# risc0/zeth

Measured on AMD Instinct MI355X. Metric: segments/sec, higher is better.
Workload: dtype u32

## Files before the change

### zeth_amd/csrc/common.h

```cpp
#pragma once
#include <hip/hip_runtime.h>

#include <atomic>
#include <cstdarg>
#include <cstdio>
#include <cstdlib>
#include <cstring>
#include <map>
#include <string>
#include <vector>

#include "../../include/zkhal.h"
#include "fp.h"
#include "noise.h"

namespace zkh {

inline const char* make_err(const char* fmt, ...) {
    char buf[512];
    va_list ap;
    va_start(ap, fmt);
    vsnprintf(buf, sizeof buf, fmt, ap);
    va_end(ap);
    return strdup(buf);
}
#define ZKH_HIP(expr)                                                                               \
    do {                                                                                            \
        hipError_t _e = (expr);                                                                     \
        if (_e != hipSuccess) return zkh::make_err("%s failed: %s (%s:%d)", #expr, hipGetErrorString(_e), __FILE__, __LINE__); \
    } while (0)
#define ZKH_TRY(expr)                    \
    do {                                 \
        const char* _err = (expr);       \
        if (_err) return _err;           \
    } while (0)
#define ZKH_REQUIRE(cond, ...)                         \
    do {                                               \
        if (!(cond)) return zkh::make_err(__VA_ARGS__); \
    } while (0)

constexpr int ZKH_P2_PTAB = 414;
constexpr int TW_BITS = 12;
constexpr int TW_SIZE = 1 << TW_BITS;
constexpr int TW_HI_BITS = 14;
constexpr int TW_HI_SIZE = 1 << TW_HI_BITS;
constexpr int MAX_LOG_N = TW_BITS + TW_HI_BITS;
constexpr int LDS_TW_LOG = 12;

struct DeviceTables {
    uint32_t* rc;
    uint32_t* diag;
    uint32_t* tw_fwd_lo; uint32_t* tw_fwd_hi;
    uint32_t* tw_rev_lo; uint32_t* tw_rev_hi;
    uint32_t* tile_fwd;  uint32_t* tile_rev;
    uint32_t* layer_fwd; uint32_t* layer_rev;
    uint32_t* layer_fwd_plain;
    uint32_t* shift_lo;  uint32_t* shift_hi;
};

struct ProfAgg { uint64_t calls = 0; double ms = 0; double bytes = 0; };
struct ProfPending { std::string name; hipEvent_t a, b; double bytes; };

}

struct zkh_alloc_t {
    void* ptr;
    size_t bytes;
    std::atomic<int> refs;
    bool owned;
    zkh_ctx* ctx;
    zkh_alloc_t(void* p, size_t b, int r, bool o, zkh_ctx* c) : ptr(p), bytes(b), refs(r), owned(o), ctx(c) {}
};

struct zkh_buf {
    zkh_alloc_t* a;
    size_t off, len;
    std::atomic<int> refs;
    zkh_buf(zkh_alloc_t* al, size_t o, size_t l, int r) : a(al), off(o), len(l), refs(r) {}
    uint32_t* ptr() const { return (uint32_t*)a->ptr + off; }
};

struct zkh_ctx {
    int device;
    hipStream_t stream;
    zkh::DeviceTables tab;
    uint32_t rou_fwd[28], rou_rev[28];
    uint32_t h_rc[24 * 29], h_diag[zkh::ZKH_P2_PTAB];
    std::multimap<size_t, void*> pool;
    size_t pool_bytes = 0, live_bytes = 0, peak_bytes = 0;
    bool prof = false;
    std::vector<zkh::ProfPending> pending;
    std::map<std::string, zkh::ProfAgg> agg;
    std::vector<hipEvent_t> event_pool;
    uint32_t* pinned = nullptr;
    size_t pinned_words = 0;
    size_t stage_next = 0, stage_used = 0;
    uint32_t* d_fail = nullptr;
    uint32_t* h_fail = nullptr;
    bool fail_armed = false;
    std::map<void*, size_t> host_blocks;
};

namespace zkh {

const char* pool_alloc(zkh_ctx* c, size_t bytes, void** out);
void pool_free(zkh_ctx* c, void* p, size_t bytes);
const char* new_buf(zkh_ctx* c, size_t n_words, bool zero, zkh_buf** out);
void prof_begin(zkh_ctx* c, const char* name, double bytes);
void prof_end(zkh_ctx* c);
const char* ensure_pinned(zkh_ctx* c, size_t words);
const char* resolve_noise_key(const uint32_t* key_or_null, NoiseKey* out);

inline void bind_thread(const zkh_ctx* c) { (void)hipSetDevice(c->device); }
const char* ntt_device_init(zkh_ctx* c);

struct Tmp {
    zkh_buf* b = nullptr;
    Tmp() {}
    Tmp(const Tmp&) = delete;
    Tmp& operator=(const Tmp&) = delete;
    ~Tmp() { if (b) zkh_release(b); }
    zkh_buf** out() { if (b) { zkh_release(b); b = nullptr; } return &b; }
    operator zkh_buf*() const { return b; }
    zkh_buf* operator->() const { return b; }
    explicit operator bool() const { return b != nullptr; }
};

struct ProfScope {
    zkh_ctx* c;
    ProfScope(zkh_ctx* ctx, const char* name, double bytes) : c(ctx) { bind_thread(c); if (c->prof) prof_begin(c, name, bytes); }
    ~ProfScope() { if (c->prof) prof_end(c); }
};

inline const char* last_launch_error(const char* what) {
    hipError_t e = hipGetLastError();
    if (e != hipSuccess) return make_err("launch %s: %s", what, hipGetErrorString(e));
    return nullptr;
}

// ... 8 lines not shown
```

### zeth_amd/csrc/hal.hip

```cpp
#include <algorithm>

#include "common.h"

#include <sys/random.h>
#include "poseidon2.h"
#include "../../include/zkh_poseidon2_consts.h"

using namespace zkh;

extern "C" void zkh_free_error(const char* e) { free((void*)e); }
#if ZKH_P2_CONSTS_ARE_PLACEHOLDER
extern "C" const char* zkh_version(void) { return "zkhal-mi355x 0.2.0 (gfx950; poseidon2_consts=placeholder)"; }
#elif ZKH_P2_CONSTS_ARE_DERIVED
extern "C" const char* zkh_version(void) { return "zkhal-mi355x 0.2.0 (gfx950; poseidon2_consts=derived)"; }
#else
extern "C" const char* zkh_version(void) { return "zkhal-mi355x 0.2.0 (gfx950; poseidon2_consts=upstream)"; }
#endif

namespace zkh {

const char* pool_alloc(zkh_ctx* c, size_t bytes, void** out) {
    bytes = (bytes + 255) & ~(size_t)255;
    if (bytes == 0) bytes = 256;
    auto it = c->pool.find(bytes);
    if (it != c->pool.end()) {
        *out = it->second;
        c->pool.erase(it);
        c->pool_bytes -= bytes;
    } else {
        hipError_t e = hipMalloc(out, bytes);
        if (e != hipSuccess) {
            (void)hipStreamSynchronize(c->stream);
            for (auto& kv : c->pool) (void)hipFree(kv.second);
            c->pool.clear(); c->pool_bytes = 0;
            e = hipMalloc(out, bytes);
            if (e != hipSuccess) return make_err("hipMalloc(%zu) failed: %s", bytes, hipGetErrorString(e));
        }
    }
    c->live_bytes += bytes;
    if (c->live_bytes > c->peak_bytes) c->peak_bytes = c->live_bytes;
    return nullptr;
}
void pool_free(zkh_ctx* c, void* p, size_t bytes) {
    bytes = (bytes + 255) & ~(size_t)255;
    if (bytes == 0) bytes = 256;
    c->live_bytes -= bytes;
    c->pool.emplace(bytes, p);
    c->pool_bytes += bytes;
}
const char* new_buf(zkh_ctx* c, size_t n_words, bool zero, zkh_buf** out) {
    bind_thread(c);
    void* p = nullptr;
    ZKH_TRY(pool_alloc(c, n_words * 4, &p));
    if (zero && n_words) {
        hipError_t e = hipMemsetAsync(p, 0, n_words * 4, c->stream);
        if (e != hipSuccess) return make_err("hipMemsetAsync: %s", hipGetErrorString(e));
    }
    zkh_alloc_t* a = new zkh_alloc_t(p, n_words * 4, 1, true, c);
    *out = new zkh_buf(a, 0, n_words, 1);
    return nullptr;
}
const char* ensure_pinned(zkh_ctx* c, size_t words) {
    if (c->pinned_words >= words) return nullptr;
    if (c->pinned) (void)hipHostFree(c->pinned);
    size_t w = words < 65536 ? 65536 : words;
    ZKH_HIP(hipHostMalloc((void**)&c->pinned, w * 4, hipHostMallocDefault));
    c->pinned_words = w;
    return nullptr;
}
static hipEvent_t get_event(zkh_ctx* c) {
    if (!c->event_pool.empty()) { hipEvent_t e = c->event_pool.back(); c->event_pool.pop_back(); return e; }
    hipEvent_t e;
    (void)hipEventCreate(&e);
    return e;
}
void prof_begin(zkh_ctx* c, const char* name, double bytes) {
    ProfPending p{name, get_event(c), get_event(c), bytes};
    (void)hipEventRecord(p.a, c->stream);
    c->pending.push_back(p);
}
void prof_end(zkh_ctx* c) { (void)hipEventRecord(c->pending.back().b, c->stream); }
static void prof_flush(zkh_ctx* c) {
    if (c->pending.empty()) return;
    (void)hipStreamSynchronize(c->stream);
    for (auto& p : c->pending) {
        float ms = 0;
        (void)hipEventElapsedTime(&ms, p.a, p.b);
        auto& g = c->agg[p.name];
// ... 16 lines not shown
    for (int tries = 0; tries < 4 && !ok; tries++) {
        ok = getrandom(out->k, sizeof out->k, 0) == (ssize_t)sizeof out->k;
        bool nonzero = false;
        for (int i = 0; i < 8; i++) nonzero = nonzero || out->k[i] != 0;
        ok = ok && nonzero;
    }
    ZKH_REQUIRE(ok, "OS randomness (getrandom) is unavailable: refusing to seal with a predictable blinding key");
    return nullptr;
}
extern "C" uint32_t zkh_noise_cell_host(const uint32_t noise_key[8], uint32_t group, uint32_t column, uint32_t row) {
    NoiseKey k;
    memcpy(k.k, noise_key, sizeof k.k);
    return noise_cell(k, group, column, row);
}
extern "C" void zkh_chacha_block_host(const uint32_t key[8], const uint32_t counter_nonce[4], int double_rounds, uint32_t out[16]) {
    chacha_block(key, counter_nonce[0], counter_nonce[1], counter_nonce[2], counter_nonce[3], double_rounds, out, 16);
}
static std::vector<uint32_t> powers(Fp base, size_t n) {
    std::vector<uint32_t> v(n);
    Fp cur = Fp::one();
    for (size_t i = 0; i < n; i++) { v[i] = cur.v; cur = cur * base; }
    return v;
}

}

extern "C" const char* zkh_poseidon2_set_constants(zkh_ctx* c, const uint32_t* rc, const uint32_t* diag) {
    bind_thread(c);
    std::vector<uint32_t> r(24 * 29), d(ZKH_P2_PTAB);
    for (int i = 0; i < 24 * 29; i++) r[i] = fp_encode(rc[i]).v - P;
    poseidon2_partial_table(d.data(), rc, diag);
    memcpy(c->h_rc, r.data(), sizeof c->h_rc);
    memcpy(c->h_diag, d.data(), sizeof c->h_diag);
    ZKH_HIP(hipStreamSynchronize(c->stream));
    ZKH_HIP(hipMemcpy(c->tab.rc, r.data(), r.size() * 4, hipMemcpyHostToDevice));
    ZKH_HIP(hipMemcpy(c->tab.diag, d.data(), d.size() * 4, hipMemcpyHostToDevice));
    return nullptr;
}

static const char* ctx_init_tables(zkh_ctx* c);
extern "C" const char* zkh_ctx_create(int device, const char* suite, zkh_ctx** out) {
    ZKH_REQUIRE(suite && strcmp(suite, "poseidon2") == 0, "unsupported hash suite '%s' (only poseidon2)", suite ? suite : "(null)");
    int ndev = 0;
    hipError_t e = hipGetDeviceCount(&ndev);
    ZKH_REQUIRE(e == hipSuccess && ndev > 0, "no HIP device available (%s): libzkhal_mi355x has no CPU fallback",
                e == hipSuccess ? "device count 0" : hipGetErrorString(e));
    ZKH_REQUIRE(device >= 0 && device < ndev, "device ordinal %d out of range (%d devices)", device, ndev);
    ZKH_HIP(hipSetDevice(device));
    zkh_ctx* c = new zkh_ctx();
    c->device = device;
    if (hipError_t se = hipStreamCreateWithFlags(&c->stream, hipStreamNonBlocking); se != hipSuccess) {
        delete c;
        return make_err("hipStreamCreateWithFlags: %s", hipGetErrorString(se));
    }
    if (const char* err = ctx_init_tables(c)) {
        zkh_ctx_destroy(c);
        return err;
    }
    *out = c;
    return nullptr;
}
static const char* ctx_init_tables(zkh_ctx* c) {
    Fp g = fp_encode(137);
    for (int k = 0; k <= 27; k++) {
        Fp w = fp_pow(g, 1ull << (27 - k));
        c->rou_fwd[k] = w.v;
        c->rou_rev[k] = fp_inv(w).v;
    }
    Fp wf = Fp::raw(c->rou_fwd[MAX_LOG_N]), wr = Fp::raw(c->rou_rev[MAX_LOG_N]);
    ZKH_TRY(upload(&c->tab.tw_fwd_lo, powers(wf, TW_SIZE)));
    ZKH_TRY(upload(&c->tab.tw_fwd_hi, powers(fp_pow(wf, TW_SIZE), TW_HI_SIZE)));
    ZKH_TRY(upload(&c->tab.tw_rev_lo, powers(wr, TW_SIZE)));
    ZKH_TRY(upload(&c->tab.tw_rev_hi, powers(fp_pow(wr, TW_SIZE), TW_HI_SIZE)));
    ZKH_TRY(upload(&c->tab.tile_fwd, powers(Fp::raw(c->rou_fwd[LDS_TW_LOG]), 1 << (LDS_TW_LOG - 1))));
    ZKH_TRY(upload(&c->tab.tile_rev, powers(Fp::raw(c->rou_rev[LDS_TW_LOG]), 1 << (LDS_TW_LOG - 1))));
    {
        std::vector<uint32_t> lf(1 << LDS_TW_LOG, R1), lr(1 << LDS_TW_LOG, R1);
        for (int j = 1; j <= LDS_TW_LOG; j++) {
            auto pf = powers(Fp::raw(c->rou_fwd[j]), (size_t)1 << (j - 1)), pr = powers(Fp::raw(c->rou_rev[j]), (size_t)1 << (j - 1));
            for (size_t e = 0; e < pf.size(); e++) { lf[((size_t)1 << (j - 1)) + e] = pf[e]; lr[((size_t)1 << (j - 1)) + e] = pr[e]; }
        }
        ZKH_TRY(upload(&c->tab.layer_fwd, lf));
        ZKH_TRY(upload(&c->tab.layer_rev, lr));
        for (auto& w : lf) w = mont_reduce((uint64_t)w);
        ZKH_TRY(upload(&c->tab.layer_fwd_plain, lf));
    }
    Fp three = fp_encode(3);
    ZKH_TRY(upload(&c->tab.shift_lo, powers(three, TW_SIZE)));
    ZKH_TRY(upload(&c->tab.shift_hi, powers(fp_pow(three, TW_SIZE), TW_HI_SIZE)));
    ZKH_TRY(upload(&c->tab.rc, std::vector<uint32_t>(24 * 29)));
    ZKH_TRY(upload(&c->tab.diag, std::vector<uint32_t>(ZKH_P2_PTAB)));
    ZKH_TRY(zkh_poseidon2_set_constants(c, ZKH_P2_ROUND_CONSTANTS, ZKH_P2_M_INT_DIAG));
    ZKH_TRY(ntt_device_init(c));
    ZKH_HIP(hipMalloc((void**)&c->d_fail, 8));
    ZKH_HIP(hipMemsetAsync(c->d_fail, 0, 8, c->stream));
    ZKH_HIP(hipHostMalloc((void**)&c->h_fail, 8, hipHostMallocDefault));
    c->h_fail[0] = c->h_fail[1] = 0;
    return nullptr;
}
extern "C" const char* zkh_ctx_trim(zkh_ctx* c) {
    bind_thread(c);
    ZKH_HIP(hipStreamSynchronize(c->stream));
    for (auto& kv : c->pool) (void)hipFree(kv.second);
    c->pool.clear(); c->pool_bytes = 0;
    return nullptr;
}
extern "C" void zkh_ctx_memory(const zkh_ctx* c, size_t* live, size_t* cached, size_t* peak) {
    if (live) *live = c->live_bytes;
    if (cached) *cached = c->pool_bytes;
    if (peak) *peak = c->peak_bytes;
}
extern "C" void zkh_ctx_destroy(zkh_ctx* c) {
    if (!c) return;
    (void)hipSetDevice(c->device);
    (void)hipStreamSynchronize(c->stream);
    for (auto& kv : c->pool) (void)hipFree(kv.second);
    uint32_t* t[] = {c->tab.rc, c->tab.diag, c->tab.tw_fwd_lo, c->tab.tw_fwd_hi, c->tab.tw_rev_lo, c->tab.tw_rev_hi,
                     c->tab.tile_fwd, c->tab.tile_rev, c->tab.shift_lo, c->tab.shift_hi, c->tab.layer_fwd, c->tab.layer_rev, c->tab.layer_fwd_plain};
    for (auto p : t) (void)hipFree(p);
    for (auto& p : c->pending) { (void)hipEventDestroy(p.a); (void)hipEventDestroy(p.b); }
    for (auto ev : c->event_pool) (void)hipEventDestroy(ev);
    if (c->pinned) (void)hipHostFree(c->pinned);
    if (c->d_fail) (void)hipFree(c->d_fail);
    if (c->h_fail) (void)hipHostFree(c->h_fail);
    for (auto& kv : c->host_blocks) (void)hipHostFree(kv.first);
    (void)hipStreamDestroy(c->stream);
    delete c;
}
static const char* check_device_fail(zkh_ctx* c) {
    if (!c->fail_armed) return nullptr;
    c->fail_armed = false;
    const uint32_t code = c->h_fail[0], detail = c->h_fail[1];
    if (!code) return nullptr;
    (void)hipMemsetAsync(c->d_fail, 0, 8, c->stream);
    switch (code) {
    case 1: return make_err("combos_prepare_regs: register %u has size 0 or more than `cycles` words (found on the device; the call's combos are unchanged)", detail);
    case 2: return make_err("combos_prepare_regs: register %u names a combo beyond combo_count (found on the device; the call's combos are unchanged)", detail);
    case 3: return make_err("combos_prepare_regs: the register sizes add up to %u U coefficients (+ %d of the check polynomial), more than coeff_u holds (found on the device; the call's combos are unchanged)", detail, ZKH_CHECK_SIZE);
    default: return make_err("a kernel reported failure code %u (%u)", code, detail);
    }
}
static const char* sync_checked(zkh_ctx* c) {
    if (c->fail_armed) ZKH_HIP(hipMemcpyAsync(c->h_fail, c->d_fail, 8, hipMemcpyDeviceToHost, c->stream));
    ZKH_HIP(hipStreamSynchronize(c->stream));
    c->stage_used = 0;
    return check_device_fail(c);
}
extern "C" const char* zkh_sync(zkh_ctx* c) {
    bind_thread(c);
    return sync_checked(c);
}
extern "C" void* zkh_ctx_stream(zkh_ctx* c) { return (void*)c->stream; }

extern "C" const char* zkh_alloc(zkh_ctx* c, const char*, size_t n, int zero, zkh_buf** out) {
    return new_buf(c, n, zero != 0, out);
}
namespace zkh {
constexpr size_t STAGE_SLOT_WORDS = 16384, STAGE_SLOTS = 64;
const char* h2d(zkh_ctx* c, uint32_t* dst, const uint32_t* host, size_t n) {
    if (!n) return nullptr;
    bind_thread(c);
    if (n <= STAGE_SLOT_WORDS) {
        ZKH_TRY(ensure_pinned(c, STAGE_SLOT_WORDS * STAGE_SLOTS));
        if (c->stage_used == STAGE_SLOTS) ZKH_TRY(sync_checked(c));
        uint32_t* slot = c->pinned + (size_t)c->stage_next * STAGE_SLOT_WORDS;
        memcpy(slot, host, n * 4);
        ZKH_HIP(hipMemcpyAsync(dst, slot, n * 4, hipMemcpyHostToDevice, c->stream));
        c->stage_next = (c->stage_next + 1) % STAGE_SLOTS;
        c->stage_used++;
        return nullptr;
    }
    ZKH_HIP(hipMemcpyAsync(dst, host, n * 4, hipMemcpyHostToDevice, c->stream));
    return sync_checked(c);
}
}
extern "C" const char* zkh_copy_from(zkh_ctx* c, const char*, const uint32_t* host, size_t n, zkh_buf** out) {
    ZKH_TRY(new_buf(c, n, false, out));
    return h2d(c, (*out)->ptr(), host, n);
}
extern "C" const char* zkh_wrap(zkh_ctx* c, void* dptr, size_t n, zkh_buf** out) {
    zkh_alloc_t* a = new zkh_alloc_t(dptr, n * 4, 1, false, c);
    *out = new zkh_buf(a, 0, n, 1);
    return nullptr;
}
extern "C" const char* zkh_slice(zkh_buf* b, size_t off, size_t n, zkh_buf** out) {
    ZKH_REQUIRE(n <= b->len && off <= b->len - n, "slice [%zu, +%zu) out of range (size %zu)", off, n, b->len);
    b->a->refs.fetch_add(1, std::memory_order_relaxed);
    *out = new zkh_buf(b->a, b->off + off, n, 1);
    return nullptr;
}
extern "C" void zkh_retain(zkh_buf* b) { b->refs.fetch_add(1, std::memory_order_relaxed); }
extern "C" void zkh_release(zkh_buf* b) {
    if (!b || b->refs.fetch_sub(1, std::memory_order_acq_rel) > 1) return;
    zkh_alloc_t* a = b->a;
    if (a->refs.fetch_sub(1, std::memory_order_acq_rel) == 1) {
        if (a->owned) pool_free(a->ctx, a->ptr, a->bytes);
        delete a;
    }
    delete b;
}
extern "C" size_t zkh_size(const zkh_buf* b) { return b->len; }
// ... 313 lines not shown
```

### zeth_amd/csrc/ntt.hip

```cpp
#include "common.h"

using namespace zkh;

namespace {

constexpr int NTT_THREADS = 256;

struct PassParams {
    const uint32_t* in;
    uint32_t* out;
    size_t in_col_stride;
    size_t out_col_stride;
    uint32_t log_n;
    uint32_t L, R;
    uint32_t log_t;
    uint32_t expand_bits;
    uint32_t first_layer;
    uint32_t twiddle;
    uint32_t scale;
    uint32_t zk_shift;
    const uint32_t* tile_tw;
    const uint32_t* layer_tw;
    const uint32_t* tw_lo;
    const uint32_t* tw_hi;
    const uint32_t* sh_lo;
    const uint32_t* sh_hi;
    uint32_t tiles_per_col;
    uint32_t lazy;
    uint32_t lazy_comp;
    uint32_t shift16[16];
};

template <bool INVERSE>
__global__ __launch_bounds__(NTT_THREADS) void k_ntt_pass(PassParams p) {
    extern __shared__ __attribute__((aligned(16))) uint32_t tile[];
    const uint32_t T = 1u << p.log_t, rows = 1u << p.R, elems = rows << p.log_t;
    const uint32_t tid = threadIdx.x;
    const uint32_t tile_id = xcd_remap(blockIdx.x, p.tiles_per_col);
    const uint32_t col = blockIdx.y;
    const uint32_t ltiles = 1u << (p.L - p.log_t);
    const uint32_t a = tile_id >> (p.L - p.log_t), lt = tile_id & (ltiles - 1);
    const size_t base = ((size_t)a << (p.L + p.R)) + ((size_t)lt << p.log_t);
    const uint32_t l0 = lt << p.log_t;
    const uint32_t* in = p.in + (size_t)col * p.in_col_stride;
    uint32_t* out = p.out + (size_t)col * p.out_col_stride;
    const uint32_t tw_shift = MAX_LOG_N - (p.L + p.R);

    for (uint32_t e = tid; e < elems; e += NTT_THREADS) {
        const uint32_t m = e >> p.log_t, t = e & (T - 1);
        const size_t gi = base + ((size_t)m << p.L) + t;
        uint32_t v = in[gi >> p.expand_bits];
        if (!INVERSE && p.twiddle) {
            const uint32_t r = __brev(m) >> (32 - p.R);
            const uint32_t ex = ((l0 + t) * r) << tw_shift;
            const uint32_t w = mul_mod(p.tw_lo[ex & (TW_SIZE - 1)], p.tw_hi[ex >> TW_BITS]);
            v = mul_mod(v, w);
        }
        tile[e] = v;
    }
    __syncthreads();

    const uint32_t half_elems = elems >> 1;
    if (INVERSE) {
        for (uint32_t j = p.R; j >= 1; j--) {
            const uint32_t hb = j - 1;
            for (uint32_t q = tid; q < half_elems; q += NTT_THREADS) {
                const uint32_t t = q & (T - 1), mm = q >> p.log_t;
                const uint32_t low = mm & ((1u << hb) - 1), m = ((mm >> hb) << j) | low;
                const uint32_t i0 = (m << p.log_t) | t, i1 = i0 + (1u << (hb + p.log_t));
                const uint32_t x = tile[i0], y = tile[i1];
                const uint32_t w = p.tile_tw[low << (LDS_TW_LOG - j)];
                tile[i0] = add_mod(x, y);
                tile[i1] = mul_mod(x - y + P, w);
            }
            __syncthreads();
        }
    } else {
        for (uint32_t j = p.first_layer; j <= p.R; j++) {
            const uint32_t hb = j - 1;
            for (uint32_t q = tid; q < half_elems; q += NTT_THREADS) {
                const uint32_t t = q & (T - 1), mm = q >> p.log_t;
                const uint32_t low = mm & ((1u << hb) - 1), m = ((mm >> hb) << j) | low;
                const uint32_t i0 = (m << p.log_t) | t, i1 = i0 + (1u << (hb + p.log_t));
// ... 73 lines not shown
                const int low = i0 & ((1 << hb) - 1), i1 = i0 + (1 << hb);
                const uint32_t w = low ? p.tile_tw[(uint32_t)low << (LDS_TW_LOG - j)] : 0u;
#pragma unroll
                for (int c = 0; c < 4; c++) {
                    const uint32_t x = v[i0][c], y = low ? mul_mod(v[i1][c], w) : v[i1][c];
                    v[i0][c] = add_mod(x, y);
                    v[i1][c] = sub_mod(x, y);
                }
            }
        }
    } else {
#pragma unroll
        for (int j = R; j >= 1; j--) {
            const int hb = j - 1;
#pragma unroll
            for (int i0 = 0; i0 < N; i0++) {
                if (i0 & (1 << hb)) continue;
                const int low = i0 & ((1 << hb) - 1), i1 = i0 + (1 << hb);
                const uint32_t w = low ? p.tile_tw[(uint32_t)low << (LDS_TW_LOG - j)] : 0u;
#pragma unroll
                for (int c = 0; c < 4; c++) {
                    const uint32_t x = v[i0][c], y = v[i1][c];
                    v[i0][c] = add_mod(x, y);
                    v[i1][c] = low ? mul_mod(x - y + P, w) : sub_mod(x, y);
                }
            }
        }
        four_step();
    }
#pragma unroll
    for (int m = 0; m < N; m++) *(uint4*)(out + ((size_t)m << p.L)) = make_uint4(v[m][0], v[m][1], v[m][2], v[m][3]);
}

__global__ void k_zk_shift(uint32_t* io, size_t total, uint32_t log_n, const uint32_t* sh_lo, const uint32_t* sh_hi) {
    size_t i = (size_t)blockIdx.x * blockDim.x + threadIdx.x;
    if (i >= total) return;
    const uint32_t pos = (uint32_t)(i & (((size_t)1 << log_n) - 1));
    const uint32_t ex = log_n ? __brev(pos) >> (32 - log_n) : 0;
    io[i] = mul_mod(io[i], mul_mod(sh_lo[ex & (TW_SIZE - 1)], sh_hi[ex >> TW_BITS]));
}

constexpr int BR_H = 5;
__global__ __launch_bounds__(256) void k_bit_reverse_tiled(uint32_t* io, uint32_t log_n, size_t col_stride) {
    __shared__ uint32_t ta[1 << (2 * BR_H)], tb[1 << (2 * BR_H)];
    const uint32_t mid_bits = log_n - 2 * BR_H;
    const uint32_t mid = blockIdx.x;
    const uint32_t rmid = mid_bits ? __brev(mid) >> (32 - mid_bits) : 0;
    if (rmid < mid) return;
    uint32_t* col = io + (size_t)blockIdx.y * col_stride;
    const uint32_t H = 1u << BR_H;
    for (uint32_t e = threadIdx.x; e < H * H; e += blockDim.x) {
        const uint32_t hi = e >> BR_H, lo = e & (H - 1);
        ta[e] = col[((size_t)hi << (log_n - BR_H)) | ((size_t)mid << BR_H) | lo];
        if (rmid != mid) tb[e] = col[((size_t)hi << (log_n - BR_H)) | ((size_t)rmid << BR_H) | lo];
    }
    __syncthreads();
    for (uint32_t e = threadIdx.x; e < H * H; e += blockDim.x) {
        const uint32_t hi2 = e >> BR_H, lo2 = e & (H - 1);
        const uint32_t shi = __brev(lo2) >> (32 - BR_H), slo = __brev(hi2) >> (32 - BR_H);
        const uint32_t src = (shi << BR_H) | slo;
        col[((size_t)hi2 << (log_n - BR_H)) | ((size_t)rmid << BR_H) | lo2] = ta[src];
        if (rmid != mid) col[((size_t)hi2 << (log_n - BR_H)) | ((size_t)mid << BR_H) | lo2] = tb[src];
    }
}
__global__ void k_bit_reverse_small(uint32_t* io, uint32_t log_n, size_t count) {
    size_t g = (size_t)blockIdx.x * blockDim.x + threadIdx.x;
    size_t n = (size_t)1 << log_n;
    if (g >= n * count) return;
    uint32_t i = (uint32_t)(g & (n - 1));
    uint32_t r = log_n ? __brev(i) >> (32 - log_n) : 0;
    if (i < r) {
        uint32_t* col = io + (g - i);
        uint32_t x = col[i], y = col[r];
        col[i] = y; col[r] = x;
    }
}


template <int LOGR, bool INVERSE, bool BASE0, int J_LO, bool LAZY = false>
__device__ __forceinline__ void radix_layers(uint32_t (&v)[1 << LOGR], const uint32_t* __restrict__ ltab,
                                             const uint32_t base_low, const int first_b) {
    constexpr int N = 1 << LOGR;
    if (!INVERSE && LAZY) {
#pragma unroll
        for (int b = 0; b < LOGR; b++) {
            if (b < first_b) continue;
            const uint32_t* tw = ltab + (1u << (J_LO + b - 1));
#pragma unroll
            for (int kk = 0; kk < (1 << b); kk++) {
                const bool unit = BASE0 && kk == 0;
                const int32_t w = (int32_t)(unit ? 1u : tw[base_low + ((uint32_t)kk << (J_LO - 1))]), nw = -w;
#pragma unroll
                for (int hi = 0; hi < (N >> (b + 1)); hi++) {
                    const int k = (hi << (b + 1)) | kk;
                    const int64_t x = (int64_t)(int32_t)v[k];
                    const int32_t y = (int32_t)v[k + (1 << b)];
                    v[k] = (uint32_t)smont_reduce(BASE0 ? mad_i64_k(y, w, x) : mad_i64(y, w, x));
                    v[k + (1 << b)] = (uint32_t)smont_reduce(BASE0 ? mad_i64_k(y, nw, x) : mad_i64(y, nw, x));
                }
            }
        }
    } else if (INVERSE) {
#pragma unroll
        for (int b = LOGR - 1; b >= 0; b--) {
            const uint32_t* tw = ltab + (1u << (J_LO + b - 1));
#pragma unroll
            for (int kk = 0; kk < (1 << b); kk++) {
                const bool unit = BASE0 && kk == 0;
                const uint32_t w = unit ? 0u : tw[base_low + ((uint32_t)kk << (J_LO - 1))];
#pragma unroll
                for (int hi = 0; hi < (N >> (b + 1)); hi++) {
                    const int k = (hi << (b + 1)) | kk;
                    const uint32_t x = v[k], y = v[k + (1 << b)];
                    v[k] = add_mod(x, y);
                    v[k + (1 << b)] = unit ? sub_mod(x, y) : mul_mod(x - y + P, w);
                }
            }
        }
    } else {
#pragma unroll
        for (int b = 0; b < LOGR; b++) {
            if (b < first_b) continue;
            const uint32_t* tw = ltab + (1u << (J_LO + b - 1));
#pragma unroll
            for (int kk = 0; kk < (1 << b); kk++) {
                const bool unit = BASE0 && kk == 0;
                const uint32_t w = unit ? 0u : tw[base_low + ((uint32_t)kk << (J_LO - 1))];
#pragma unroll
                for (int hi = 0; hi < (N >> (b + 1)); hi++) {
                    const int k = (hi << (b + 1)) | kk;
                    const uint32_t x = v[k], y = unit ? v[k + (1 << b)] : mul_mod(v[k + (1 << b)], w);
                    v[k] = add_mod(x, y);
                    v[k + (1 << b)] = sub_mod(x, y);
                }
            }
        }
    }
}

template <bool INVERSE, bool LAZY = false>
__global__ __launch_bounds__(256) void k_ntt_low12(PassParams p) {
    __shared__ __attribute__((aligned(16))) uint32_t lds[4096];
    const uint32_t tid = threadIdx.x;
    const uint32_t tile = xcd_remap(blockIdx.x, p.tiles_per_col);
    const size_t base = (size_t)tile << 12;
    const uint32_t* in = p.in + (size_t)blockIdx.y * p.in_col_stride;
    uint32_t* out = p.out + (size_t)blockIdx.y * p.out_col_stride;
    const uint32_t* __restrict__ ltab = p.layer_tw;
    const uint32_t hi = tid >> 4, low = tid & 15;
    uint32_t v[16];
    if (INVERSE) {
#pragma unroll
        for (int k = 0; k < 16; k++) v[k] = in[base + k * 256 + tid];
        radix_layers<4, true, false, 9>(v, ltab, tid, 0);
#pragma unroll
        for (int k = 0; k < 16; k++) lds[k * 256 + tid] = v[k];
        __syncthreads();
#pragma unroll
        for (int k = 0; k < 16; k++) v[k] = lds[hi * 256 + k * 16 + low];
        radix_layers<4, true, false, 5>(v, ltab, low, 0);
#pragma unroll
        for (int k = 0; k < 16; k++) lds[hi * 256 + k * 16 + low] = v[k];
        __syncthreads();
#pragma unroll
        for (int q = 0; q < 4; q++) {
            const uint4 w = ((const uint4*)lds)[tid * 4 + q];
            v[4 * q] = w.x; v[4 * q + 1] = w.y; v[4 * q + 2] = w.z; v[4 * q + 3] = w.w;
        }
        radix_layers<4, true, true, 1>(v, ltab, 0, 0);
        const size_t pos0 = base + (size_t)tid * 16;
        if (p.zk_shift) {
            const uint32_t ex = __brev((uint32_t)pos0) >> (32 - p.log_n);
            const uint32_t b = mul_mod(p.sh_lo[ex & (TW_SIZE - 1)], p.sh_hi[ex >> TW_BITS]);
#pragma unroll
            for (int k = 0; k < 16; k++) v[k] = mul_mod(mul_mod(v[k], b), p.shift16[k]);
        } else if (p.scale) {
#pragma unroll
            for (int k = 0; k < 16; k++) v[k] = mul_mod(v[k], p.scale);
        }
#pragma unroll
        for (int q = 0; q < 4; q++) ((uint4*)(out + pos0))[q] = make_uint4(v[4 * q], v[4 * q + 1], v[4 * q + 2], v[4 * q + 3]);
    } else {
        const size_t pos0 = base + (size_t)tid * 16;
        if (p.expand_bits == 0) {
// ... 118 lines not shown
                radix_layers<2, false, true, 1, LAZY>(u, ltab, 0, 0);
#pragma unroll
                for (int k = 0; k < 4; k++) lds[(m0 + k) * TW + t] = u[k];
            }
            __syncthreads();
#pragma unroll
            for (int k = 0; k < 16; k++) v[k] = lds[(hi * 64 + k * 4 + low) * TW + t];
            radix_layers<4, false, false, 3, LAZY>(v, ltab, low, 0);
#pragma unroll
            for (int k = 0; k < 16; k++) lds[(hi * 64 + k * 4 + low) * TW + t] = v[k];
            __syncthreads();
#pragma unroll
            for (int k = 0; k < 16; k++) v[k] = lds[(k * 64 + g) * TW + t];
            radix_layers<4, false, false, 7, LAZY>(v, ltab, g, 0);
#pragma unroll
            for (int k = 0; k < 16; k++) TILE_OUT(k * 64 + g) = LAZY ? canon((int32_t)v[k]) : v[k];
        }
    } else {
        if (INVERSE) {
#pragma unroll
            for (int k = 0; k < 16; k++) v[k] = TILE_IN(k * 16 + g);
            radix_layers<4, true, false, 5>(v, ltab, g, 0);
#pragma unroll
            for (int k = 0; k < 16; k++) lds[(k * 16 + g) * TW + t] = v[k];
            __syncthreads();
#pragma unroll
            for (int k = 0; k < 16; k++) v[k] = lds[(g * 16 + k) * TW + t];
            radix_layers<4, true, true, 1>(v, ltab, 0, 0);
#pragma unroll
            for (int k = 0; k < 16; k++) {
                uint32_t x = mul_mod(v[k], tw[k]);
                if (p.scale) x = mul_mod(x, p.scale);
                TILE_OUT(g * 16 + k) = x;
            }
        } else {
#pragma unroll
            for (int k = 0; k < 16; k++) {
                const uint32_t x = TILE_IN(g * 16 + k);
                v[k] = LAZY ? (uint32_t)smont((int32_t)x, (int32_t)tw[k]) : mul_mod(x, tw[k]);
            }
            radix_layers<4, false, true, 1, LAZY>(v, ltab, 0, 0);
#pragma unroll
            for (int k = 0; k < 16; k++) lds[(g * 16 + k) * TW + t] = v[k];
            __syncthreads();
#pragma unroll
            for (int k = 0; k < 16; k++) v[k] = lds[(k * 16 + g) * TW + t];
            radix_layers<4, false, false, 5, LAZY>(v, ltab, g, 0);
#pragma unroll
            for (int k = 0; k < 16; k++) TILE_OUT(k * 16 + g) = LAZY ? canon((int32_t)v[k]) : v[k];
        }
    }
}
#undef TILE_IN
#undef TILE_OUT

struct Pass { uint32_t L, R; };
std::vector<Pass> plan_passes(uint32_t log_n) {
    std::vector<Pass> v;
    if (log_n <= 12) { v.push_back({0, log_n}); return v; }
    if (log_n < 18) {
        const uint32_t low = (log_n + 1) / 2;
        v.push_back({0, low});
        v.push_back({low, log_n - low});
        return v;
    }
    const uint32_t rem = log_n - 12;
    v.push_back({0, 12});
    if (rem == 8 || rem == 10 || rem <= 7) v.push_back({12, rem});
    else if (rem == 9) { v.push_back({12, 8}); v.push_back({20, 1}); }
    else if (rem == 11 || rem == 12) { v.push_back({12, 8}); v.push_back({20, rem - 8}); }
    else { v.push_back({12, 10}); v.push_back({22, rem - 10}); }
    return v;
}

const char* run_transform(zkh_ctx* c, bool inverse, const uint32_t* in, size_t in_col_stride, uint32_t* out,
                          size_t out_col_stride, uint32_t log_n, size_t count, uint32_t expand_bits, bool zk, const char* name) {
    ZKH_REQUIRE(log_n <= (uint32_t)MAX_LOG_N, "%s: transform size 2^%u exceeds the supported 2^%d", name, log_n, MAX_LOG_N);
    ZKH_REQUIRE(count <= 65535, "%s: too many columns (%zu)", name, count);
    std::vector<Pass> passes = plan_passes(log_n);
    const size_t n = (size_t)1 << log_n;
    Fp ninv = fp_inv(fp_encode((uint32_t)(n % P)));
    const size_t npass = passes.size();
    const bool lazy = !inverse && npass == 2 && passes[0].R == 12 && (passes[1].R == 8 || passes[1].R == 10) && expand_bits <= 4;
    const uint32_t lazy_comp = lazy ? fp_pow(Fp::raw(R2), passes[0].R - expand_bits + passes[1].R).v : 0;
    for (size_t pi = 0; pi < npass; pi++) {
        const Pass ps = inverse ? passes[npass - 1 - pi] : passes[pi];
        PassParams p{};
        const bool first = pi == 0, last = pi + 1 == npass;
        p.in = first ? in : out;
        p.in_col_stride = first ? in_col_stride : out_col_stride;
        p.out = out; p.out_col_stride = out_col_stride;
        p.log_n = log_n; p.L = ps.L; p.R = ps.R;
        const bool reg_high = ps.L >= 4 && (ps.R == 8 || ps.R == 10);
        p.log_t = ps.L == 0 ? 0 : (ps.L < 4 ? ps.L : 4);
        if (ps.L != 0 && !reg_high && ps.R < 12) p.log_t = std::max<uint32_t>(p.log_t, std::min<uint32_t>(ps.L, 12 - ps.R));
        while (p.R + p.log_t > 14 && p.log_t > 0) p.log_t--;
        p.expand_bits = (!inverse && first) ? expand_bits : 0;
        p.first_layer = (!inverse && first) ? expand_bits + 1 : 1;
        p.twiddle = ps.L != 0;
        p.scale = (inverse && last) ? ninv.v : 0;
        p.zk_shift = (inverse && last && zk) ? 1 : 0;
        p.lazy = lazy; p.lazy_comp = lazy_comp;
        p.tile_tw = inverse ? c->tab.tile_rev : c->tab.tile_fwd;
        p.layer_tw = inverse ? c->tab.layer_rev : (lazy ? c->tab.layer_fwd_plain : c->tab.layer_fwd);
        p.tw_lo = inverse ? c->tab.tw_rev_lo : c->tab.tw_fwd_lo;
        p.tw_hi = inverse ? c->tab.tw_rev_hi : c->tab.tw_fwd_hi;
        p.sh_lo = c->tab.shift_lo; p.sh_hi = c->tab.shift_hi;
        if (p.zk_shift && log_n >= 4) {
            const Fp three = fp_encode(3);
            for (uint32_t k = 0; k < 16; k++)
                p.shift16[k] = (ninv * fp_pow(three, (uint64_t)(bitrev32(k) >> 28) << (log_n - 4))).v;
        }
        p.tiles_per_col = (uint32_t)(n >> (p.R + p.log_t));
        const size_t lds = ((size_t)4 << (p.R + p.log_t));
        dim3 grid(p.tiles_per_col, (unsigned)count);
        const double alg_bytes = pi == 0 ? 4.0 * count * (double)(((size_t)1 << log_n) >> expand_bits) + 4.0 * count * (double)n : 0.0;
        const bool scale_here = p.scale != 0;
        const bool k_low = ps.L == 0 && ps.R == 12 && p.expand_bits <= 4;
        const bool k_h10 = !k_low && ps.L >= 4 && p.log_t == 4 && ps.R == 10 && !(scale_here && p.zk_shift);
        const bool k_h8 = !k_low && !k_h10 && ps.L >= 4 && p.log_t == 4 && ps.R == 8 && !(scale_here && p.zk_shift);
        const bool k_top = !k_low && !k_h10 && !k_h8 && ps.L >= 12 && ps.L + ps.R == log_n && ps.R >= 1 && ps.R <= 4 && p.twiddle &&
                           p.expand_bits == 0 && p.first_layer == 1 && !scale_here && !p.zk_shift;
        const std::string pname = std::string(name) + (k_low ? ":k_ntt_low12" : k_h10 ? ":k_ntt_high10" : k_h8 ? ":k_ntt_high8" : k_top ? ":k_ntt_top" : ":k_ntt_pass");
        ProfScope prof(c, pname.c_str(), alg_bytes);
        if (ps.L == 0 && ps.R == 12 && p.expand_bits <= 4) {
            if (inverse) k_ntt_low12<true><<<grid, 256, 0, c->stream>>>(p);
            else if (lazy) k_ntt_low12<false, true><<<grid, 256, 0, c->stream>>>(p);
            else k_ntt_low12<false><<<grid, 256, 0, c->stream>>>(p);
        } else if (ps.L >= 4 && p.log_t == 4 && ps.R == 10 && !(scale_here && p.zk_shift)) {
            if (inverse) k_ntt_high<10, true><<<grid, 1024, lds, c->stream>>>(p);
            else if (lazy) k_ntt_high<10, false, true><<<grid, 1024, lds, c->stream>>>(p);
            else k_ntt_high<10, false><<<grid, 1024, lds, c->stream>>>(p);
        } else if (ps.L >= 4 && p.log_t == 4 && ps.R == 8 && !(scale_here && p.zk_shift)) {
            if (inverse) k_ntt_high<8, true><<<grid, 256, lds, c->stream>>>(p);
            else if (lazy) k_ntt_high<8, false, true><<<grid, 256, lds, c->stream>>>(p);
            else k_ntt_high<8, false><<<grid, 256, lds, c->stream>>>(p);
        } else if (k_top) {
            const dim3 tg((unsigned)(((size_t)1 << ps.L) >> 10), (unsigned)count);
            switch (ps.R * 2 + (inverse ? 1 : 0)) {
            case 2: k_ntt_top<1, false><<<tg, 256, 0, c->stream>>>(p); break;
            case 3: k_ntt_top<1, true><<<tg, 256, 0, c->stream>>>(p); break;
            case 4: k_ntt_top<2, false><<<tg, 256, 0, c->stream>>>(p); break;
            case 5: k_ntt_top<2, true><<<tg, 256, 0, c->stream>>>(p); break;
            case 6: k_ntt_top<3, false><<<tg, 256, 0, c->stream>>>(p); break;
            case 7: k_ntt_top<3, true><<<tg, 256, 0, c->stream>>>(p); break;
            case 8: k_ntt_top<4, false><<<tg, 256, 0, c->stream>>>(p); break;
            default: k_ntt_top<4, true><<<tg, 256, 0, c->stream>>>(p); break;
            }
        } else if (inverse) k_ntt_pass<true><<<grid, NTT_THREADS, lds, c->stream>>>(p);
        else k_ntt_pass<false><<<grid, NTT_THREADS, lds, c->stream>>>(p);
        ZKH_TRY(last_launch_error(name));
    }
    return nullptr;
}

}

const char* zkh::ntt_device_init(zkh_ctx* c) {
    bind_thread(c);
    ZKH_HIP(hipFuncSetAttribute((const void*)k_ntt_high<10, true>, hipFuncAttributeMaxDynamicSharedMemorySize, 65536));
    ZKH_HIP(hipFuncSetAttribute((const void*)k_ntt_high<10, false>, hipFuncAttributeMaxDynamicSharedMemorySize, 65536));
    ZKH_HIP(hipFuncSetAttribute((const void*)k_ntt_high<10, false, true>, hipFuncAttributeMaxDynamicSharedMemorySize, 65536));
    return nullptr;
}

static const char* interpolate_impl(zkh_ctx* c, zkh_buf* io, size_t count, bool zk, const char* name) {
    ZKH_REQUIRE(count && io->len % count == 0, "%s: size %zu not a multiple of count %zu", name, io->len, count);
    const size_t n = io->len / count;
    const uint32_t log_n = log2_ceil(n);
    ZKH_REQUIRE(((size_t)1 << log_n) == n, "%s: column length %zu is not a power of two", name, n);
    return run_transform(c, true, io->ptr(), n, io->ptr(), n, log_n, count, 0, zk, name);
}
extern "C" const char* zkh_batch_interpolate_ntt(zkh_ctx* c, zkh_buf* io, size_t count) {
    return interpolate_impl(c, io, count, false, "batch_interpolate_ntt");
}
extern "C" const char* zkh_batch_interpolate_ntt_zk_shift(zkh_ctx* c, zkh_buf* io, size_t count) {
    return interpolate_impl(c, io, count, true, "batch_interpolate_ntt_zk_shift");
}
extern "C" const char* zkh_batch_interpolate_ntt_from(zkh_ctx* c, zkh_buf* out, const zkh_buf* in, size_t count, int zk_shift) {
    ZKH_REQUIRE(count && in->len % count == 0 && out->len == in->len, "batch_interpolate_ntt_from: shape mismatch");
    const size_t n = in->len / count;
    const uint32_t log_n = log2_ceil(n);
    ZKH_REQUIRE(((size_t)1 << log_n) == n, "batch_interpolate_ntt_from: column length %zu is not a power of two", n);
    return run_transform(c, true, in->ptr(), n, out->ptr(), n, log_n, count, 0, zk_shift != 0, "batch_interpolate_ntt_from");
}
extern "C" const char* zkh_batch_expand_into_evaluate_ntt(zkh_ctx* c, zkh_buf* out, const zkh_buf* in, size_t count,
                                                          size_t expand_bits) {
// ... 36 lines not shown
```

Measured before the change: 42.80.

## Fuse pairs of lazy NTT butterfly layers to halve Montgomery reductions

Reworks the lazy forward NTT radix layers to process two butterfly layers at once. The first layer's sums stay as unreduced 64-bit accumulators and get folded into the second layer's multiply-add, so only one signed Montgomery reduction happens per two layers. A new twiddle table holds centered plain and Montgomery-form twiddles for this, and the compensation power of R is recomputed from the new reduction count. This cuts the ALU work spent on reductions, at the cost of wider intermediate values and extra twiddle loads, with some overflow risk in the unreduced sums.

```diff
diff --git a/zeth_amd/csrc/common.h b/zeth_amd/csrc/common.h
--- a/zeth_amd/csrc/common.h
+++ b/zeth_amd/csrc/common.h
@@ -54,7 +54,7 @@
     uint32_t* tw_rev_lo; uint32_t* tw_rev_hi;
     uint32_t* tile_fwd;  uint32_t* tile_rev;
     uint32_t* layer_fwd; uint32_t* layer_rev;
-    uint32_t* layer_fwd_plain;
+    uint32_t* layer_fwd_lazy;
     uint32_t* shift_lo;  uint32_t* shift_hi;
 };
 
diff --git a/zeth_amd/csrc/hal.hip b/zeth_amd/csrc/hal.hip
--- a/zeth_amd/csrc/hal.hip
+++ b/zeth_amd/csrc/hal.hip
@@ -4,6 +4,7 @@
 
 #include <sys/random.h>
 #include "poseidon2.h"
+#include "ntt_lazy.h"
 #include "../../include/zkh_poseidon2_consts.h"
 
 using namespace zkh;
@@ -186,8 +187,10 @@
         }
         ZKH_TRY(upload(&c->tab.layer_fwd, lf));
         ZKH_TRY(upload(&c->tab.layer_rev, lr));
-        for (auto& w : lf) w = mont_reduce((uint64_t)w);
-        ZKH_TRY(upload(&c->tab.layer_fwd_plain, lf));
+        static_assert(LAZY_TAB_LOG == LDS_TW_LOG, "the lazy table covers the per-layer tables");
+        std::vector<uint32_t> lz(LAZY_TAB_WORDS);
+        lazy_layer_table(lz.data(), lf.data());
+        ZKH_TRY(upload(&c->tab.layer_fwd_lazy, lz));
     }
     Fp three = fp_encode(3);
     ZKH_TRY(upload(&c->tab.shift_lo, powers(three, TW_SIZE)));
@@ -220,7 +223,7 @@
     (void)hipStreamSynchronize(c->stream);
     for (auto& kv : c->pool) (void)hipFree(kv.second);
     uint32_t* t[] = {c->tab.rc, c->tab.diag, c->tab.tw_fwd_lo, c->tab.tw_fwd_hi, c->tab.tw_rev_lo, c->tab.tw_rev_hi,
-                     c->tab.tile_fwd, c->tab.tile_rev, c->tab.shift_lo, c->tab.shift_hi, c->tab.layer_fwd, c->tab.layer_rev, c->tab.layer_fwd_plain};
+                     c->tab.tile_fwd, c->tab.tile_rev, c->tab.shift_lo, c->tab.shift_hi, c->tab.layer_fwd, c->tab.layer_rev, c->tab.layer_fwd_lazy};
     for (auto p : t) (void)hipFree(p);
     for (auto& p : c->pending) { (void)hipEventDestroy(p.a); (void)hipEventDestroy(p.b); }
     for (auto ev : c->event_pool) (void)hipEventDestroy(ev);
diff --git a/zeth_amd/csrc/ntt.hip b/zeth_amd/csrc/ntt.hip
--- a/zeth_amd/csrc/ntt.hip
+++ b/zeth_amd/csrc/ntt.hip
@@ -1,4 +1,5 @@
 #include "common.h"
+#include "ntt_lazy.h"
 
 using namespace zkh;
 
@@ -238,24 +239,7 @@
                                              const uint32_t base_low, const int first_b) {
     constexpr int N = 1 << LOGR;
     if (!INVERSE && LAZY) {
-#pragma unroll
-        for (int b = 0; b < LOGR; b++) {
-            if (b < first_b) continue;
-            const uint32_t* tw = ltab + (1u << (J_LO + b - 1));
-#pragma unroll
-            for (int kk = 0; kk < (1 << b); kk++) {
-                const bool unit = BASE0 && kk == 0;
-                const int32_t w = (int32_t)(unit ? 1u : tw[base_low + ((uint32_t)kk << (J_LO - 1))]), nw = -w;
-#pragma unroll
-                for (int hi = 0; hi < (N >> (b + 1)); hi++) {
-                    const int k = (hi << (b + 1)) | kk;
-                    const int64_t x = (int64_t)(int32_t)v[k];
-                    const int32_t y = (int32_t)v[k + (1 << b)];
-                    v[k] = (uint32_t)smont_reduce(BASE0 ? mad_i64_k(y, w, x) : mad_i64(y, w, x));
-                    v[k + (1 << b)] = (uint32_t)smont_reduce(BASE0 ? mad_i64_k(y, nw, x) : mad_i64(y, nw, x));
-                }
-            }
-        }
+        lazy_layers<LOGR, BASE0, J_LO>(v, ltab, base_low, first_b);
     } else if (INVERSE) {
 #pragma unroll
         for (int b = LOGR - 1; b >= 0; b--) {
@@ -540,7 +524,8 @@
     Fp ninv = fp_inv(fp_encode((uint32_t)(n % P)));
     const size_t npass = passes.size();
     const bool lazy = !inverse && npass == 2 && passes[0].R == 12 && (passes[1].R == 8 || passes[1].R == 10) && expand_bits <= 4;
-    const uint32_t lazy_comp = lazy ? fp_pow(Fp::raw(R2), passes[0].R - expand_bits + passes[1].R).v : 0;
+    const uint32_t lazy_reds = lazy ? lazy_reductions(4, expand_bits) + 2 * lazy_reductions(4, 0) + lazy_reductions(passes[1].R, 0) : 0;
+    const uint32_t lazy_comp = lazy ? fp_pow(Fp::raw(R2), lazy_reds).v : 0;
     for (size_t pi = 0; pi < npass; pi++) {
         const Pass ps = inverse ? passes[npass - 1 - pi] : passes[pi];
         PassParams p{};
@@ -560,7 +545,7 @@
         p.zk_shift = (inverse && last && zk) ? 1 : 0;
         p.lazy = lazy; p.lazy_comp = lazy_comp;
         p.tile_tw = inverse ? c->tab.tile_rev : c->tab.tile_fwd;
-        p.layer_tw = inverse ? c->tab.layer_rev : (lazy ? c->tab.layer_fwd_plain : c->tab.layer_fwd);
+        p.layer_tw = inverse ? c->tab.layer_rev : (lazy ? c->tab.layer_fwd_lazy : c->tab.layer_fwd);
         p.tw_lo = inverse ? c->tab.tw_rev_lo : c->tab.tw_fwd_lo;
         p.tw_hi = inverse ? c->tab.tw_rev_hi : c->tab.tw_fwd_hi;
         p.sh_lo = c->tab.shift_lo; p.sh_hi = c->tab.shift_hi;
diff --git a/zeth_amd/csrc/ntt_lazy.h b/zeth_amd/csrc/ntt_lazy.h
--- /dev/null
+++ b/zeth_amd/csrc/ntt_lazy.h
@@ -0,0 +1,94 @@
+#pragma once
+#include "fp.h"
+
+#ifndef ZKH_LAZY_SUM
+#define ZKH_LAZY_SUM(t) ((void)0)
+#endif
+
+namespace zkh {
+
+constexpr int LAZY_TAB_LOG = 12;
+constexpr uint32_t LAZY_TAB_MONT = 1u << LAZY_TAB_LOG;
+constexpr uint32_t LAZY_TAB_WORDS = 2u << LAZY_TAB_LOG;
+
+inline void lazy_layer_table(uint32_t* out, const uint32_t* layer_fwd) {
+    for (uint32_t i = 0; i < LAZY_TAB_MONT; i++) {
+        out[i] = (uint32_t)center(mont_reduce((uint64_t)layer_fwd[i]));
+        out[LAZY_TAB_MONT + i] = (uint32_t)center(layer_fwd[i]);
+    }
+}
+
+template <bool UNIFORM>
+ZKH_HD int64_t lazy_mad(int32_t a, int32_t w, int64_t acc) {
+    if constexpr (UNIFORM) return mad_i64_k(a, w, acc);
+    else return mad_i64(a, w, acc);
+}
+ZKH_HD int32_t lazy_reduce(int64_t t) {
+    ZKH_LAZY_SUM(t);
+    return smont_reduce(t);
+}
+
+template <bool UNIFORM>
+ZKH_HD void lazy_single(uint32_t& v0, uint32_t& v1, int32_t w) {
+    const int64_t x = (int64_t)(int32_t)v0;
+    const int32_t y = (int32_t)v1, nw = -w;
+    v0 = (uint32_t)lazy_reduce(lazy_mad<UNIFORM>(y, w, x));
+    v1 = (uint32_t)lazy_reduce(lazy_mad<UNIFORM>(y, nw, x));
+}
+
+template <bool UNIFORM>
+ZKH_HD void lazy_pair(uint32_t& v0, uint32_t& v1, uint32_t& v2, uint32_t& v3, int32_t wa, int32_t wb0, int32_t wb1) {
+    const int32_t nwa = -wa, nwb0 = -wb0, nwb1 = -wb1;
+    const int64_t x0 = (int64_t)(int32_t)v0, x2 = (int64_t)(int32_t)v2;
+    const int32_t x1 = (int32_t)v1, x3 = (int32_t)v3;
+    const int32_t u2 = lazy_reduce(lazy_mad<UNIFORM>(x3, wa, x2));
+    const int32_t u3 = lazy_reduce(lazy_mad<UNIFORM>(x3, nwa, x2));
+    const int64_t sp = lazy_mad<UNIFORM>(x1, wa, x0), sm = lazy_mad<UNIFORM>(x1, nwa, x0);
+    v0 = (uint32_t)lazy_reduce(lazy_mad<UNIFORM>(u2, wb0, sp));
+    v2 = (uint32_t)lazy_reduce(lazy_mad<UNIFORM>(u2, nwb0, sp));
+    v1 = (uint32_t)lazy_reduce(lazy_mad<UNIFORM>(u3, wb1, sm));
+    v3 = (uint32_t)lazy_reduce(lazy_mad<UNIFORM>(u3, nwb1, sm));
+}
+
+ZKH_HD uint32_t lazy_reductions(uint32_t logr, uint32_t first_b) {
+    const uint32_t live = first_b < logr ? logr - first_b : 0;
+    return (live + 1) / 2;
+}
+
+template <int LOGR, bool BASE0, int J_LO>
+ZKH_HD void lazy_layers(uint32_t (&v)[1 << LOGR], const uint32_t* __restrict__ ltab, const uint32_t base_low, const int first_b) {
+    static_assert(LOGR % 2 == 0, "lazy rounds hold an even number of layers");
+    constexpr int N = 1 << LOGR;
+#pragma unroll
+    for (int b = 0; b < LOGR; b += 2) {
+        const uint32_t* twa = ltab + (1u << (J_LO + b - 1));
+        const uint32_t* twb = ltab + LAZY_TAB_MONT + (1u << (J_LO + b));
+        if (b >= first_b) {
+#pragma unroll
+            for (int kk = 0; kk < (1 << b); kk++) {
+                const uint32_t e = base_low + ((uint32_t)kk << (J_LO - 1));
+                const int32_t wa = (BASE0 && kk == 0) ? 1 : (int32_t)twa[e];
+                const int32_t wb0 = (BASE0 && kk == 0) ? (int32_t)R1 : (int32_t)twb[e];
+                const int32_t wb1 = (int32_t)twb[e + ((1u << b) << (J_LO - 1))];
+#pragma unroll
+                for (int hi = 0; hi < (N >> (b + 2)); hi++) {
+                    const int k = (hi << (b + 2)) | kk;
+                    lazy_pair<BASE0>(v[k], v[k + (1 << b)], v[k + (2 << b)], v[k + (3 << b)], wa, wb0, wb1);
+                }
+            }
+        } else if (b + 1 >= first_b) {
+            const uint32_t* tw1 = ltab + (1u << (J_LO + b));
+#pragma unroll
+            for (int kk = 0; kk < (2 << b); kk++) {
+                const int32_t w = (BASE0 && kk == 0) ? 1 : (int32_t)tw1[base_low + ((uint32_t)kk << (J_LO - 1))];
+#pragma unroll
+                for (int hi = 0; hi < (N >> (b + 2)); hi++) {
+                    const int k = (hi << (b + 2)) | kk;
+                    lazy_single<BASE0>(v[k], v[k + (2 << b)], w);
+                }
+            }
+        }
+    }
+}
+
+}
```

After: 43.58, median of 6. 1.8% higher.
